# DaLi-Jack/G4Splat

Hardware: AMD Instinct MI355X
Metric: rasterized Gaussians/s fwd+bwd @1600x1200 (higher is better)
Workload: dtype f32

## Files before the change

g4splat_amd/csrc/api.hip:

```cpp
#include <stdarg.h>
#include <stdio.h>
#include <stdlib.h>
#include <string.h>

#include <atomic>
#include <mutex>
#include <vector>

#include "g4s_internal.h"

using namespace g4s;

namespace {
thread_local char t_err[512] = "";
}

namespace g4s {
void clear_error() { t_err[0] = 0; }
int fail(int code, const char* fmt, ...) {
    va_list ap;
    va_start(ap, fmt);
    vsnprintf(t_err, sizeof(t_err), fmt, ap);
    va_end(ap);
    return code;
// ... 267 lines not shown
        geom = align_ptr(geom);
        float* rec = (float*)(geom + GL.rec);
        uint32_t* tiles_touched = (uint32_t*)(geom + GL.tiles_touched);
        uint32_t* keys_a = (uint32_t*)(geom + GL.keys_a);
        uint32_t* keys_b = (uint32_t*)(geom + GL.keys_b);
        uint32_t* vals_a = (uint32_t*)(geom + GL.vals_a);
        uint32_t* vals_b = (uint32_t*)(geom + GL.vals_b);
        uint32_t* block_sums = (uint32_t*)(geom + GL.block_sums);
        uint32_t* block_offs = (uint32_t*)(geom + GL.block_offs);
        uint32_t* d_total = (uint32_t*)(geom + GL.total);
        int* const radii = c.radii ? c.radii : (int*)(geom + GL.internal_radii);

        PreprocessArgs pa{};
        pa.P = P; pa.D = c.D; pa.M = c.M; pa.W = c.width; pa.H = c.height; pa.tiles_x = tiles_x; pa.tiles_y = tiles_y;
        pa.means3D = c.means3D; pa.scales = c.scales; pa.rotations = c.rotations; pa.opacities = c.opacities; pa.shs = c.shs;
        pa.transMat_precomp = c.transMat_precomp; pa.colors_precomp = c.colors_precomp;
        pa.viewmatrix = c.viewmatrix; pa.projmatrix = c.projmatrix; pa.cam_pos = c.cam_pos;
        pa.scale_modifier = c.scale_modifier;
        pa.shs_rest = c.shs_rest;
        pa.sh_vec16 = (c.shs != nullptr && c.shs_rest == nullptr && c.M == 16 && !misaligned(c.shs, 16));
        pa.no_fastpath = opt(OPT_NO_FASTPATH) != 0;
        pa.rec = rec; pa.clamped = (uint8_t*)(geom + GL.clamped); pa.tiles_touched = tiles_touched; pa.radii = radii;
        pa.tight_rect = (uint2*)(geom + GL.tight_rect);
        uint32_t* const k_first = presized ? keys_b : keys_a;
        uint32_t* const k_other = presized ? keys_a : keys_b;
        uint32_t* const v_first = presized ? vals_b : vals_a;
        uint32_t* const v_other = presized ? vals_a : vals_b;
        pa.depth_keys = k_other;
        pa.ref_block_sums = (uint32_t*)(geom + GL.ref_block_sums);
        pa.idx_block_sums = (uint32_t*)(geom + GL.idx_block_sums);
        pa.vis_block_sums = (uint32_t*)(geom + GL.vis_block_sums);
        pa.key_min_blocks = (uint32_t*)(geom + GL.key_min_blocks);
        pa.key_max_blocks = (uint32_t*)(geom + GL.key_max_blocks);
        { ProfScope ps(PF_PREPROCESS_FWD, stream); launch_preprocess_fwd(pa, stream); }
        CHECK_LAUNCH("preprocess_fwd");

        uint32_t* idx_block_offs = (uint32_t*)(geom + GL.idx_block_offs);
        uint32_t* vis_block_offs = (uint32_t*)(geom + GL.vis_block_offs);
        uint32_t* h_total = nullptr;
        uint32_t* h_total_dev = nullptr;
        hipEvent_t totals_ready = nullptr;
        if (!presized) {
            h_total = pinned_word();
            h_total_dev = h_total ? pinned_word_device(h_total) : nullptr;
            if (!h_total || !h_total_dev) return fail(G4S_ERR_HIP, "hipHostMalloc / hipHostGetDevicePointer failed");
            totals_ready = readback_event();
            if (!totals_ready) return fail(G4S_ERR_HIP, "hipEventCreate failed");
        }
        { ProfScope ps(PF_COUNT_SCAN, stream);
          launch_scan_totals(pa.idx_block_sums, idx_block_offs, pa.ref_block_sums, pa.vis_block_sums, vis_block_offs,
                             d_total, GL.nblocks, ranges, tiles * 2, stream, presized ? (uint32_t)c.capacity : 0xFFFFFFFFu,
                             h_total_dev, presized ? c.status_dev : nullptr, pa.key_min_blocks, pa.key_max_blocks); }
        CHECK_LAUNCH("scan totals");
        if (!presized) {
            HIP_TRY(hipEventRecord(totals_ready, stream));
        }

        const uint32_t* d_V = d_total + 2;
        const uint32_t* d_key_min = d_total + 5;
        uint32_t* sort_hist = (uint32_t*)(geom + GL.hist);
        uint32_t* sort_bins = (uint32_t*)(geom + GL.bin_total);
        int cur;
        {
            ProfScope ps(PF_DEPTH_SORT, stream);
            launch_slots_and_compact(P, tiles_touched, idx_block_offs, rec, k_other, vis_block_offs, k_first, v_first,
                                     GL.nblocks, stream);
            cur = presized ? radix_sort_u32_pairs(k_first, k_other, v_first, v_other, P, sort_hist, sort_bins, stream, d_V)
                           : radix_sort_depth_low(k_first, k_other, v_first, v_other, P, sort_hist, sort_bins, stream, d_V,
                                                  d_key_min);
        }
        CHECK_LAUNCH("depth sort");

        int R_binned, V_emit, nblocks_v;
        const uint32_t* d_counts = nullptr;
        const uint32_t* d_nbinned = nullptr;
        if (!presized) {
            HIP_TRY(hipEventSynchronize(totals_ready));
            if (h_total[1] > 0x7FFFFFFFu) return fail(G4S_ERR_INVALID_ARGUMENT, "num_rendered overflows int");
            R = (int)h_total[1];
            R_binned = (int)h_total[0];
            V_emit = (int)h_total[2];
            nblocks_v = (V_emit + 255) / 256;
            if (V_emit > 0 && ((uint64_t)h_total[4] - h_total[3]) >> DEPTH_SORT_LOW_BITS) {
                ProfScope ps(PF_DEPTH_SORT, stream);
// ... 294 lines not shown
```

g4splat_amd/csrc/binning.hip:

```cpp
#include "g4s_internal.h"
#include "g4s_device.h"

namespace g4s {


template <typename K>
__device__ __forceinline__ uint32_t radix_digit(K key, uint32_t base, int shift, uint32_t mask) {
    return (uint32_t)((K)(key - (K)base) >> shift) & mask;
}

template <typename K, int ITEMS, int BITS>
__global__ void __launch_bounds__(256) radix_hist_kernel(const K* __restrict__ keys, int n, int shift, uint32_t mask,
                                                         uint32_t* __restrict__ hist, int nblocks,
                                                         const uint32_t* __restrict__ d_n,
                                                         const uint32_t* __restrict__ key_base) {
    constexpr int BINS = 1 << BITS;
    __shared__ uint32_t h[BINS];
    constexpr int TK = 256 * ITEMS;
    const int block = (int)blockIdx.x;
    if (d_n != nullptr) {
        n = (int)*d_n;
        nblocks = (n + TK - 1) / TK;
        if (block >= nblocks) return;
    }
// ... 202 lines not shown
    return cur ^ 1;
}

int radix_sort_u64_keys(uint64_t* a, uint64_t* b, int n, int begin_bit, int end_bit, uint32_t* hist,
                        uint32_t* bin_total, hipStream_t s, const uint32_t* d_n) {
    if (n <= 0 || end_bit <= begin_bit) return 0;
    const int bits = end_bit - begin_bit, passes = (bits + 7) / 8, per = (bits + passes - 1) / passes;
    int cur = 0;
    for (int shift = begin_bit; shift < end_bit; shift += per) {
        const int nb = per < end_bit - shift ? per : end_bit - shift;
        if (cur == 0)
            radix_pass<uint64_t, false, SORT_ITEMS_U64>(a, b, nullptr, nullptr, n, shift, nb, hist, bin_total, s, d_n);
        else
            radix_pass<uint64_t, false, SORT_ITEMS_U64>(b, a, nullptr, nullptr, n, shift, nb, hist, bin_total, s, d_n);
        cur ^= 1;
    }
    return cur;
}


__global__ void __launch_bounds__(256) count_block_sums_kernel(int P, const uint32_t* __restrict__ gidx,
                                                               const uint32_t* __restrict__ tiles_touched,
                                                               uint32_t* __restrict__ block_sums,
                                                               uint32_t* __restrict__ rank_local,
                                                               const uint32_t* __restrict__ d_n) {
    __shared__ uint32_t sm4[4];
    if (d_n != nullptr) {
        P = (int)*d_n;
        if ((int)(blockIdx.x * 256) >= P) return;
    }
    const int r = (int)(blockIdx.x * 256 + threadIdx.x);
    uint32_t c = 0;
    if (r < P) c = tiles_touched[gidx[r]];
    uint32_t total;
    const uint32_t local = block256_excl_scan_u32(c, sm4, &total);
    if (r < P) rank_local[r] = local;
    if (threadIdx.x == 0) block_sums[blockIdx.x] = total;
}

__global__ void __launch_bounds__(1024) scan_block_sums_kernel(int nblocks, const uint32_t* __restrict__ a_sums,
                                                               uint32_t* __restrict__ a_offs,
                                                               const uint32_t* __restrict__ b_sums,
                                                               uint32_t* __restrict__ b_offs,
                                                               const uint32_t* __restrict__ ref_sums,
                                                               uint32_t* __restrict__ total_a, uint32_t* __restrict__ total_b,
                                                               uint32_t* __restrict__ zero_ptr, int zero_words,
                                                               const uint32_t* __restrict__ d_n, uint32_t capacity,
                                                               uint32_t* __restrict__ host_out,
                                                               uint32_t* __restrict__ status_out,
                                                               const uint32_t* __restrict__ kmin_blocks,
                                                               const uint32_t* __restrict__ kmax_blocks) {
    __shared__ uint32_t wa[16], wb[16], wr[16], wlo[16], whi[16];
    const int t = (int)threadIdx.x;
    for (int i = t; i < zero_words; i += 1024) zero_ptr[i] = 0u;
    if (d_n != nullptr) nblocks = (int)((*d_n + 255u) / 256u);
    const int seg = (nblocks + 1023) / 1024;
    const int b = imin_(nblocks, t * seg), e = imin_(nblocks, b + seg);
    uint32_t sa = 0, sb = 0, sr = 0, klo = 0xFFFFFFFFu, khi = 0u;
    for (int i = b; i < e; i++) {
        sa += a_sums[i];
        if (b_sums) sb += b_sums[i];
        if (ref_sums) sr += ref_sums[i];
        if (kmin_blocks) {
            klo = min(klo, kmin_blocks[i]);
            khi = max(khi, kmax_blocks[i]);
        }
    }
    if (kmin_blocks) {
        klo = ~wave_max_u32_full_wave(~klo);
        khi = wave_max_u32_full_wave(khi);
    }
    const uint32_t ia = wave_incl_scan_u32(sa), ib = wave_incl_scan_u32(sb), ir = wave_incl_scan_u32(sr);
    if ((t & 63) == 63) {
        wa[t >> 6] = ia;
        wb[t >> 6] = ib;
        wr[t >> 6] = ir;
        wlo[t >> 6] = klo;
        whi[t >> 6] = khi;
    }
    __syncthreads();
    uint32_t base_a = 0, base_b = 0, all_a = 0, all_b = 0, all_r = 0;
    for (int w = 0; w < 16; w++) {
        if (w < (t >> 6)) { base_a += wa[w]; base_b += wb[w]; }
        all_a += wa[w];
        all_b += wb[w];
        all_r += wr[w];
    }
    uint32_t run_a = base_a + ia - sa, run_b = base_b + ib - sb;
    for (int i = b; i < e; i++) {
        a_offs[i] = run_a;
        run_a += a_sums[i];
        if (b_sums) { b_offs[i] = run_b; run_b += b_sums[i]; }
    }
    if (t == 0) {
        total_a[0] = all_a;
        total_a[1] = all_r;
        if (kmin_blocks) {
            uint32_t lo = 0xFFFFFFFFu, hi = 0u;
            for (int w = 0; w < 16; w++) { lo = min(lo, wlo[w]); hi = max(hi, whi[w]); }
            if (lo > hi) lo = hi = 0u;
            total_a[5] = lo;
            total_a[6] = hi;
            if (host_out != nullptr) { host_out[3] = lo; host_out[4] = hi; }
        }
        if (b_sums) {
            total_b[0] = all_b;
            total_b[1] = all_a < capacity ? all_a : capacity;
            total_b[2] = all_a > capacity ? 1u : 0u;
        }
        if (status_out != nullptr) {
            status_out[0] = all_r;
            status_out[1] = all_a;
            status_out[2] = all_b;
            status_out[3] = all_a > capacity ? 1u : 0u;
        }
        if (host_out != nullptr) {
            host_out[0] = all_a;
            host_out[1] = all_r;
            host_out[2] = all_b;
        }
    }
}

void launch_count_scan(int P, const uint32_t* gidx_sorted, const uint32_t* tiles_touched, uint32_t* block_sums,
                       uint32_t* block_offs, uint32_t* rank_local, uint32_t* total, int nblocks, hipStream_t s,
                       const uint32_t* d_n) {
    hipLaunchKernelGGL(count_block_sums_kernel, dim3(nblocks), dim3(256), 0, s, P, gidx_sorted, tiles_touched,
                       block_sums, rank_local, d_n);
    hipLaunchKernelGGL(scan_block_sums_kernel, dim3(1), dim3(1024), 0, s, nblocks, block_sums, block_offs,
                       (const uint32_t*)nullptr, (uint32_t*)nullptr, (const uint32_t*)nullptr, total, (uint32_t*)nullptr,
                       (uint32_t*)nullptr, 0, d_n, 0xFFFFFFFFu, (uint32_t*)nullptr, (uint32_t*)nullptr,
                       (const uint32_t*)nullptr, (const uint32_t*)nullptr);
}

constexpr int EMIT_SLOTS = 1024;
__global__ void __launch_bounds__(256) emit_kernel(int V, uint32_t R_b, int tiles_x,
                                                   const uint32_t* __restrict__ gidx,
                                                   const uint32_t* __restrict__ block_offs, int nblocks_v,
                                                   const uint32_t* __restrict__ rank_local,
                                                   const uint2* __restrict__ tight_rect,
                                                   uint64_t* __restrict__ entries, uint8_t* __restrict__ qhit,
                                                   uint8_t* __restrict__ rec_flag,
                                                   const uint32_t* __restrict__ d_counts) {
    __shared__ uint32_t s_off[EMIT_SLOTS + 4];
    __shared__ uint32_t s_idx[EMIT_SLOTS + 4];
    __shared__ uint32_t s_rect[EMIT_SLOTS + 4];
    __shared__ uint32_t s_rect2[EMIT_SLOTS + 4];
    __shared__ uint32_t s_nr;
    const int t = (int)threadIdx.x;
    if (d_counts != nullptr) {
        V = (int)d_counts[0];
        R_b = d_counts[1];
        nblocks_v = (V + 255) / 256;
    }
    const uint32_t w0 = blockIdx.x * (uint32_t)EMIT_SLOTS;
    if (w0 >= R_b) return;
    const uint32_t w1 = min(w0 + (uint32_t)EMIT_SLOTS, R_b);
    {
        const uint32_t o = w0 + 4u * (uint32_t)t;
        if (o + 4u <= w1) {
            *reinterpret_cast<uint32_t*>(qhit + o) = 0u;
            *reinterpret_cast<uint32_t*>(rec_flag + o) = 0u;
        } else {
            for (uint32_t i = o; i < w1; i++) { qhit[i] = 0; rec_flag[i] = 0; }
        }
    }
    if (t == 0) s_nr = 0;
    int lo = 0, n = nblocks_v;
    while (n > 1) {
        const int S = (n + 255) / 256;
        const int j = lo + t * S;
        const int c = __syncthreads_count(t * S < n && block_offs[j] <= w0);
        lo += (c - 1) * S;
        n = imin_(S, n - (c - 1) * S);
    }
    const int g = lo;
    const uint32_t goff = block_offs[g];
    int r_first;
    {
        const int r = 256 * g + t;
        const int c = __syncthreads_count(r < V && goff + rank_local[r] <= w0);
        r_first = 256 * g + c - 1;
    }
    for (int i = t; i <= EMIT_SLOTS; i += 256) {
        const int r = r_first + i;
        if (r >= V) break;
        const uint32_t off = block_offs[r >> 8] + rank_local[r];
        if (off >= w1) break;
        const uint32_t idx = gidx[r];
        const uint2 tr = tight_rect[idx];
        s_off[i] = off;
        s_idx[i] = idx;
        s_rect[i] = tr.x;
        s_rect2[i] = tr.y;
        atomicMax(&s_nr, (uint32_t)i + 1u);
    }
    __syncthreads();
    const int nr = (int)s_nr;
    const int steps = 32 - __builtin_clz((uint32_t)nr | 1u);
    for (uint32_t o = w0 + (uint32_t)t; o < w1; o += 256) {
        int a = 0, b = nr - 1;
        for (int it = 0; it < steps; it++) {
            const int mid = (a + b + 1) >> 1;
            if (s_off[mid] <= o) a = mid; else b = mid - 1;
        }
        const uint32_t k = o - s_off[a];
        const uint32_t w = s_rect2[a];
        const uint32_t rx0 = s_rect[a] & 0xFFFFu, ry0 = s_rect[a] >> 16;
        const uint32_t ty = k / w, tx = k - ty * w;
        const uint64_t tile = (uint64_t)((ry0 + ty) * (uint32_t)tiles_x + rx0 + tx);
        entries[o] = (tile << ENTRY_TILE_SHIFT) | (uint64_t)s_idx[a];
    }
}

__global__ void __launch_bounds__(256) slots_and_compact_kernel(int P, const uint32_t* __restrict__ tiles_touched,
                                                                const uint32_t* __restrict__ idx_block_offs,
                                                                float* __restrict__ rec,
                                                                const uint32_t* __restrict__ depth_keys,
                                                                const uint32_t* __restrict__ vis_block_offs,
                                                                uint32_t* __restrict__ keys_out,
                                                                uint32_t* __restrict__ idx_out) {
    __shared__ uint32_t sm4[4], sm4b[4];
    const int idx = (int)(blockIdx.x * 256 + threadIdx.x);
    const uint32_t c = idx < P ? tiles_touched[idx] : 0u;
    uint32_t total;
    const uint32_t slot = block256_excl_scan_u32(c, sm4, &total);
    const uint32_t local = block256_excl_scan_u32(c > 0 ? 1u : 0u, sm4b, &total);
    if (c > 0) {
        rec[(size_t)idx * REC_FLOATS + 2] = __uint_as_float(idx_block_offs[blockIdx.x] + slot);
        const uint32_t dst = vis_block_offs[blockIdx.x] + local;
        keys_out[dst] = depth_keys[idx];
        idx_out[dst] = (uint32_t)idx;
    }
}
void launch_slots_and_compact(int P, const uint32_t* tiles_touched, const uint32_t* idx_block_offs, float* rec,
                              const uint32_t* depth_keys, const uint32_t* vis_block_offs, uint32_t* keys_out,
                              uint32_t* idx_out, int nblocks, hipStream_t s) {
    hipLaunchKernelGGL(slots_and_compact_kernel, dim3(nblocks), dim3(256), 0, s, P, tiles_touched, idx_block_offs, rec,
                       depth_keys, vis_block_offs, keys_out, idx_out);
}

void launch_scan_totals(const uint32_t* idx_block_sums, uint32_t* idx_block_offs, const uint32_t* ref_block_sums,
                        const uint32_t* vis_block_sums, uint32_t* vis_block_offs, uint32_t* total, int nblocks,
                        uint32_t* zero_ptr, int zero_words, hipStream_t s, uint32_t capacity, uint32_t* host_out,
                        uint32_t* status_out, const uint32_t* key_min_blocks, const uint32_t* key_max_blocks) {
    hipLaunchKernelGGL(scan_block_sums_kernel, dim3(1), dim3(1024), 0, s, nblocks, idx_block_sums, idx_block_offs,
                       vis_block_sums, vis_block_offs, ref_block_sums, total, total + 2, zero_ptr, zero_words,
                       (const uint32_t*)nullptr, capacity, host_out, status_out, key_min_blocks, key_max_blocks);
}

void launch_emit(int V, uint32_t R_b, int tiles_x, const uint32_t* gidx_sorted, const uint32_t* block_offs,
                 int nblocks_v, const uint32_t* rank_local, const uint2* tight_rect, uint64_t* entries,
                 uint8_t* qhit, uint8_t* rec_flag, hipStream_t s, const uint32_t* d_counts) {
    if (R_b == 0) return;
    hipLaunchKernelGGL(emit_kernel, dim3((R_b + EMIT_SLOTS - 1) / EMIT_SLOTS), dim3(256), 0, s, V, R_b, tiles_x,
                       gidx_sorted, block_offs, nblocks_v, rank_local, tight_rect, entries, qhit, rec_flag, d_counts);
}

__global__ void __launch_bounds__(256) tile_ranges_kernel(int R, const uint64_t* __restrict__ entries,
                                                          uint32_t* __restrict__ ranges, const uint32_t* __restrict__ d_n) {
    if (d_n != nullptr) R = (int)*d_n;
    const int i0 = (int)(blockIdx.x * 256 + threadIdx.x) * 4;
    if (i0 >= R) return;
    uint64_t e[4];
    if (i0 + 4 <= R) {
        const ulonglong2 a = *reinterpret_cast<const ulonglong2*>(entries + i0);
        const ulonglong2 b = *reinterpret_cast<const ulonglong2*>(entries + i0 + 2);
        e[0] = a.x; e[1] = a.y; e[2] = b.x; e[3] = b.y;
    } else {
#pragma unroll
        for (int k = 0; k < 4; k++) e[k] = entries[i0 + k < R ? i0 + k : R - 1];
    }
    uint32_t prev = i0 > 0 ? entry_tile(entries[i0 - 1]) : 0xFFFFFFFFu;
#pragma unroll
    for (int k = 0; k < 4; k++) {
        const int i = i0 + k;
        if (i >= R) break;
        const uint32_t cur = entry_tile(e[k]);
        if (i == 0) {
            ranges[2 * cur] = 0;
        } else if (cur != prev) {
            ranges[2 * prev + 1] = (uint32_t)i;
            ranges[2 * cur] = (uint32_t)i;
        }
        if (i == R - 1) ranges[2 * cur + 1] = (uint32_t)R;
        prev = cur;
    }
}

constexpr int ORDER_BUCKETS = 2048;
__global__ void __launch_bounds__(1024) tile_order_kernel(int tiles, const uint32_t* __restrict__ ranges,
                                                          uint32_t* __restrict__ order, uint32_t* __restrict__ zero_word) {
    __shared__ uint32_t hist[ORDER_BUCKETS];
    __shared__ uint32_t wsum[16];
    const int t = (int)threadIdx.x;
    if (t == 0 && zero_word != nullptr) *zero_word = 0u;
    for (int i = t; i < ORDER_BUCKETS; i += 1024) hist[i] = 0;
    __syncthreads();
    auto bucket = [](uint32_t n) {
        const uint32_t b = n >> 2;
        return (uint32_t)(ORDER_BUCKETS - 1) - (b < (uint32_t)(ORDER_BUCKETS - 1) ? b : (uint32_t)(ORDER_BUCKETS - 1));
    };
    for (int i = t; i < tiles; i += 1024) atomicAdd(&hist[bucket(ranges[2 * i + 1] - ranges[2 * i])], 1u);
    __syncthreads();
    const uint32_t h0 = hist[2 * t], h1 = hist[2 * t + 1];
    const uint32_t inc = wave_incl_scan_u32(h0 + h1);
    if ((t & 63) == 63) wsum[t >> 6] = inc;
    __syncthreads();
    uint32_t base = 0;
    for (int w = 0; w < (t >> 6); w++) base += wsum[w];
    const uint32_t ex = base + inc - (h0 + h1);
    __syncthreads();
    hist[2 * t] = ex;
    hist[2 * t + 1] = ex + h0;
    __syncthreads();
    for (int i = t; i < tiles; i += 1024) order[atomicAdd(&hist[bucket(ranges[2 * i + 1] - ranges[2 * i])], 1u)] = (uint32_t)i;
}
void launch_tile_order(int tiles, const uint32_t* ranges, uint32_t* tile_order, hipStream_t s, uint32_t* zero_word) {
    hipLaunchKernelGGL(tile_order_kernel, dim3(1), dim3(1024), 0, s, tiles, ranges, tile_order, zero_word);
}

void launch_tile_ranges(int R, const uint64_t* entries, uint32_t* ranges, hipStream_t s, const uint32_t* d_n) {
    if (R <= 0) return;
    hipLaunchKernelGGL(tile_ranges_kernel, dim3((R + 1023) / 1024), dim3(256), 0, s, R, entries, ranges, d_n);
}

}
```

g4splat_amd/csrc/g4s_device.h:

```cpp
#pragma once
#include <hip/hip_runtime.h>
#include <stdint.h>

#include "g4s_internal.h"

namespace g4s {

constexpr int WAVE = 64;

__device__ __forceinline__ int lane_id() { return (int)(threadIdx.x & 63); }

template <int CTRL, int ROW_MASK = 0xF, int BANK_MASK = 0xF>
__device__ __forceinline__ float dpp_f32(float v) {
    return __builtin_bit_cast(
        float, __builtin_amdgcn_update_dpp(0, __builtin_bit_cast(int, v), CTRL, ROW_MASK, BANK_MASK, false));
}
template <int CTRL, int ROW_MASK = 0xF, int BANK_MASK = 0xF>
__device__ __forceinline__ uint32_t dpp_u32(uint32_t v) {
    return (uint32_t)__builtin_amdgcn_update_dpp(0, (int)v, CTRL, ROW_MASK, BANK_MASK, false);
}

__device__ __forceinline__ void acc_fma(float& acc, float a, float b) { asm volatile("v_fmac_f32 %0, %1, %2" : "+v"(acc) : "v"(a), "v"(b)); }
__device__ __forceinline__ void acc_add(float& acc, float a) { asm volatile("v_add_f32 %0, %0, %1" : "+v"(acc) : "v"(a)); }
__device__ __forceinline__ void acc_sub(float& acc, float a) { asm volatile("v_sub_f32 %0, %0, %1" : "+v"(acc) : "v"(a)); }
// ... 92 lines not shown
        "v_permlane16_swap_b32 %3, %7"
        : "+v"(s0), "+v"(s1), "+v"(s2), "+v"(s3), "+v"(s4), "+v"(s5), "+v"(s6), "+v"(s7));
    const float r0 = s0 + s4, r1 = s1 + s5, r2 = s2 + s6, r3 = s3 + s7;
    const float k01 = b3 ? r1 : r0, g01 = b3 ? r0 : r1;
    const float k23 = b3 ? r3 : r2, g23 = b3 ? r2 : r3;
    const float x01 = k01 + dpp_f32<0x128>(g01);
    const float x23 = k23 + dpp_f32<0x128>(g23);
    const float k = b2 ? x23 : x01, g = b2 ? x01 : x23;
    float y = k + dpp_f32<0x141>(g);
    y += dpp_f32<0xB1>(y);
    y += dpp_f32<0x4E>(y);
    asm volatile("" : "+v"(y));
    return y;
}

__device__ __forceinline__ uint32_t wave_sum_u32(uint32_t v) {
    return (uint32_t)__builtin_amdgcn_readlane((int)wave_sum_to_lane63(v), 63);
}
__device__ __forceinline__ uint32_t wave_max_u32(uint32_t v) {
    for (int off = 32; off >= 1; off >>= 1) {
        uint32_t o = (uint32_t)__shfl_xor((int)v, off, 64);
        v = v > o ? v : o;
    }
    return v;
}
__device__ __forceinline__ uint32_t wave_max_u32_full_wave(uint32_t v) {
    v = max(v, dpp_u32<0xB1>(v));
    v = max(v, dpp_u32<0x4E>(v));
    v = max(v, dpp_u32<0x124>(v));
    v = max(v, dpp_u32<0x128>(v));
    v = max(v, dpp_u32<0x142, 0xA>(v));
    v = max(v, dpp_u32<0x143, 0xC>(v));
    return (uint32_t)__builtin_amdgcn_readlane((int)v, 63);
}

__device__ __forceinline__ uint32_t wave_incl_scan_u32(uint32_t v) {
    const int l = lane_id();
    for (int off = 1; off < 64; off <<= 1) {
        uint32_t o = (uint32_t)__shfl_up((int)v, off, 64);
        if (l >= off) v += o;
    }
    return v;
}

__device__ __forceinline__ uint64_t lanes_below_mask() {
    return (1ull << lane_id()) - 1ull;
}

__device__ __forceinline__ uint32_t block256_excl_scan_u32(uint32_t v, uint32_t* smem4, uint32_t* block_total) {
    const int w = (int)(threadIdx.x >> 6);
    uint32_t inc = wave_incl_scan_u32(v);
    __syncthreads();
    if (lane_id() == 63) smem4[w] = inc;
    __syncthreads();
    uint32_t s0 = smem4[0], s1 = smem4[1], s2 = smem4[2], s3 = smem4[3];
    uint32_t base = (w > 0 ? s0 : 0) + (w > 1 ? s1 : 0) + (w > 2 ? s2 : 0);
    *block_total = s0 + s1 + s2 + s3;
    return base + inc - v;
}

__device__ __forceinline__ int sat_int(float v) { return (int)v; }

struct F3 {
    float x, y, z;
};
__device__ __forceinline__ F3 mk3(float x, float y, float z) { return F3{x, y, z}; }
// ... 171 lines not shown
```

g4splat_amd/csrc/g4s_internal.h:

```cpp
#pragma once
#include <hip/hip_runtime.h>
#include <stddef.h>
#include <stdint.h>

#include "../../include/g4s_rasterizer.h"

namespace g4s {

constexpr int TILE = 16;
constexpr int REC_FLOATS = 32;
constexpr int REC_QUADS = REC_FLOATS / 4;
constexpr int BLEND_QUADS = 5;
constexpr int GRAD_FLOATS = 18;
constexpr int GRAD_STRIDE = 20;
__host__ __device__ inline void box_quadrants(float lo, float hi, int extent, uint32_t& q0, uint32_t& q1) {
    const float l = ceilf(lo), h = floorf(hi);
    const float top = (float)(extent - 1);
    q0 = 1u;
    q1 = 0u;
    if (!(l <= h) || !(h >= 0.0f) || !(l <= top)) return;
    q0 = (l > 0.0f ? (uint32_t)l : 0u) >> 3;
    q1 = (h < top ? (uint32_t)h : (uint32_t)(extent - 1)) >> 3;
}
constexpr uint32_t CULLED_KEY = 0xFFFFFFFFu;
// ... 96 lines not shown
int fail(int code, const char* fmt, ...);
int finish(hipError_t e, const char* what);
int stage_done(const char* what, hipStream_t s, bool debug = false);
inline bool misaligned(const void* p, size_t a) { return p != nullptr && ((size_t)p % a) != 0; }

enum ProfId { PF_PREPROCESS_FWD, PF_DEPTH_SORT, PF_COUNT_SCAN, PF_EMIT, PF_TILE_SORT, PF_TILE_RANGES, PF_BLEND_FWD,
              PF_BLEND_BWD, PF_PREPROCESS_BWD, PF_MAPS_FWD, PF_MAPS_BWD, PF_PHOTO_LOSS, PF_ADAM, PF_GEO_REG, PF_COUNT };
struct ProfScope {
    int id; hipStream_t s; hipEvent_t a = nullptr, b = nullptr; bool on = false;
    ProfScope(int id_, hipStream_t s_);
    ~ProfScope();
};


struct PreprocessArgs {
    int P, D, M, W, H, tiles_x, tiles_y;
    uint32_t* ref_block_sums;
    uint32_t* idx_block_sums;
    uint32_t* vis_block_sums;
    uint32_t* key_min_blocks;
    uint32_t* key_max_blocks;
    const float *means3D, *scales, *rotations, *opacities, *shs, *transMat_precomp, *colors_precomp;
    const float *viewmatrix, *projmatrix, *cam_pos;
    float scale_modifier;
    bool sh_vec16;
    bool no_fastpath;
    const float* shs_rest;
    float* rec;
    uint8_t* clamped;
    uint32_t* tiles_touched;
    uint2* tight_rect;
    int* radii;
    uint32_t* depth_keys;
};
void launch_preprocess_fwd(const PreprocessArgs& a, hipStream_t s);

int radix_sort_u32_pairs(uint32_t* keys_a, uint32_t* keys_b, uint32_t* vals_a, uint32_t* vals_b, int n,
                         uint32_t* hist, uint32_t* bin_total, hipStream_t s, const uint32_t* d_n = nullptr);
int radix_sort_depth_low(uint32_t* keys_a, uint32_t* keys_b, uint32_t* vals_a, uint32_t* vals_b, int n, uint32_t* hist,
                         uint32_t* bin_total, hipStream_t s, const uint32_t* d_n, const uint32_t* key_min);
int radix_sort_depth_top(uint32_t* keys_a, uint32_t* keys_b, uint32_t* vals_a, uint32_t* vals_b, int n, int cur,
                         uint32_t* hist, uint32_t* bin_total, hipStream_t s, const uint32_t* d_n, const uint32_t* key_min);
int radix_sort_u64_keys(uint64_t* a, uint64_t* b, int n, int begin_bit, int end_bit, uint32_t* hist,
                        uint32_t* bin_total, hipStream_t s, const uint32_t* d_n = nullptr);

void launch_count_scan(int P, const uint32_t* gidx_sorted, const uint32_t* tiles_touched, uint32_t* block_sums,
                       uint32_t* block_offs, uint32_t* rank_local, uint32_t* total, int nblocks, hipStream_t s,
                       const uint32_t* d_n = nullptr);
void launch_scan_totals(const uint32_t* idx_block_sums, uint32_t* idx_block_offs, const uint32_t* ref_block_sums,
                        const uint32_t* vis_block_sums, uint32_t* vis_block_offs, uint32_t* total, int nblocks,
                        uint32_t* zero_ptr, int zero_words, hipStream_t s, uint32_t capacity = 0xFFFFFFFFu,
                        uint32_t* host_out = nullptr, uint32_t* status_out = nullptr,
                        const uint32_t* key_min_blocks = nullptr, const uint32_t* key_max_blocks = nullptr);
void launch_slots_and_compact(int P, const uint32_t* tiles_touched, const uint32_t* idx_block_offs, float* rec,
                              const uint32_t* depth_keys, const uint32_t* vis_block_offs, uint32_t* keys_out,
                              uint32_t* idx_out, int nblocks, hipStream_t s);
void launch_emit(int V, uint32_t R_b, int tiles_x, const uint32_t* gidx_sorted, const uint32_t* block_offs,
                 int nblocks_v, const uint32_t* rank_local, const uint2* tight_rect, uint64_t* entries,
                 uint8_t* qhit, uint8_t* rec_flag, hipStream_t s, const uint32_t* d_counts);
void launch_tile_ranges(int R, const uint64_t* entries, uint32_t* ranges, hipStream_t s, const uint32_t* d_n = nullptr);
void launch_tile_order(int tiles, const uint32_t* ranges, uint32_t* tile_order, hipStream_t s, uint32_t* zero_word = nullptr);

struct BlendFwdArgs {
    int W, H, tiles_x, tiles_y;
    const uint32_t* ranges;
    const uint32_t* tile_order;
// ... 67 lines not shown
```

g4splat_amd/csrc/preprocess.hip:

```cpp
#include "g4s_internal.h"
#include "g4s_device.h"

namespace g4s {

__constant__ float c_SH_C2[5] = {1.0925484305920792f, -1.0925484305920792f, 0.31539156525252005f,
                                 -1.0925484305920792f, 0.5462742152960396f};
__constant__ float c_SH_C3[7] = {-0.5900435899266435f, 2.890611442640554f, -0.4570457994644658f,
                                 0.3731763325901154f,  -0.4570457994644658f, 1.445305721320277f,
                                 -0.5900435899266435f};
#define SH_C0 0.28209479177387814f
#define SH_C1 0.4886025119029199f

__device__ __forceinline__ void compute_transmat(F3 p, float sx, float sy, float mod, const float* R,
                                                 const float* proj, int W, int H, float* T) {
    const float s0 = mod * sx, s1 = mod * sy;
    const float Mrow[3][4] = {{R[0] * s0, R[1] * s0, R[2] * s0, 0.0f},
                              {R[3] * s1, R[4] * s1, R[5] * s1, 0.0f},
                              {p.x, p.y, p.z, 1.0f}};
    const float hw = (float)((float)W / 2.0), cw = (float)((float)(W - 1) / 2.0);
    const float hh = (float)((float)H / 2.0), ch = (float)((float)(H - 1) / 2.0);
#pragma unroll
    for (int r = 0; r < 3; r++) {
        float c[4];
#pragma unroll
// ... 255 lines not shown
            r[c] = r[c] - SH_C1 * y * sh[3 + c] + SH_C1 * z * sh[6 + c] - SH_C1 * x * sh[9 + c];
        if (deg > 1) {
            const float xx = x * x, yy = y * y, zz = z * z, xy = x * y, yz = y * z, xz = x * z;
#pragma unroll
            for (int c = 0; c < 3; c++)
                r[c] = r[c] + c_SH_C2[0] * xy * sh[12 + c] + c_SH_C2[1] * yz * sh[15 + c] +
                       c_SH_C2[2] * (2.0f * zz - xx - yy) * sh[18 + c] + c_SH_C2[3] * xz * sh[21 + c] +
                       c_SH_C2[4] * (xx - yy) * sh[24 + c];
            if (deg > 2) {
#pragma unroll
                for (int c = 0; c < 3; c++)
                    r[c] = r[c] + c_SH_C3[0] * y * (3.0f * xx - yy) * sh[27 + c] + c_SH_C3[1] * xy * z * sh[30 + c] +
                           c_SH_C3[2] * y * (4.0f * zz - xx - yy) * sh[33 + c] +
                           c_SH_C3[3] * z * (2.0f * zz - 3.0f * xx - 3.0f * yy) * sh[36 + c] +
                           c_SH_C3[4] * x * (4.0f * zz - xx - yy) * sh[39 + c] +
                           c_SH_C3[5] * z * (xx - yy) * sh[42 + c] + c_SH_C3[6] * x * (xx - 3.0f * yy) * sh[45 + c];
            }
        }
    }
    clamp_bits = 0;
#pragma unroll
    for (int c = 0; c < 3; c++) {
        r[c] += 0.5f;
        if (r[c] < 0) clamp_bits |= (1u << c);
        rgb[c] = fmaxf(r[c], 0.0f);
    }
}

template <int SH_MODE>
__global__ void __launch_bounds__(256) __attribute__((amdgpu_waves_per_eu(5, 5))) preprocess_fwd_kernel(PreprocessArgs a) {
    __shared__ __attribute__((aligned(16))) float s_cert[4][64 * CERT_SLOT_WORDS];
    __shared__ uint32_t s_cert_fail[4][64];
    const int idx = (int)(blockIdx.x * 256 + threadIdx.x);
    const bool in_range = idx < a.P;
    int radius_out = 0;
    uint32_t touched_ref = 0, touched = 0, key = CULLED_KEY, clamp_bits = 0;
    float T[9], cx, cy, opa, rgb[3];
    F3 normal;
    float4 box;
    int tx0, ty0, tx1, ty1;
    SplatAffine af;
    bool want = false;

    if (in_range) {
        const F3 p = mk3(a.means3D[3 * idx], a.means3D[3 * idx + 1], a.means3D[3 * idx + 2]);
        const F3 p_view = xform_point_4x3(p, a.viewmatrix);
        if (p_view.z > 0.2f) {
            if (a.transMat_precomp == nullptr) {
                float R[9];
                const float4 q = reinterpret_cast<const float4*>(a.rotations)[idx];
                const float2 sc = reinterpret_cast<const float2*>(a.scales)[idx];
                quat_to_rotmat(q, R);
                compute_transmat(p, sc.x, sc.y, a.scale_modifier, R, a.projmatrix, a.W, a.H, T);
                normal = xform_vec_4x3(mk3(R[6], R[7], R[8]), a.viewmatrix);
            } else {
#pragma unroll
                for (int i = 0; i < 9; i++) T[i] = a.transMat_precomp[9 * (size_t)idx + i];
                normal = mk3(0.0f, 0.0f, 1.0f);
            }
            const float cosv = -((p_view.x * normal.x + p_view.y * normal.y) + p_view.z * normal.z);
            if (cosv != 0) {
                const float mult = cosv > 0 ? 1.0f : -1.0f;
                normal = mk3(mult * normal.x, mult * normal.y, mult * normal.z);
                float ex, ey;
                if (compute_aabb(T, 3.0f, cx, cy, ex, ey)) {
                    const float radius = ceilf(fmaxf(ex, ey));
// ... 754 lines not shown
```

Baseline: 268.6 million.

## Rework binning scans, emit lookup, tile order, and move range zeroing into preprocess

Zeroing of the tile ranges buffer moves out of the single-block scan_totals kernel and into the grid-wide preprocess kernel. The block-sum scan is now chunked and wave-parallel with DPP scans instead of serial per-thread segments. The emit kernel replaces its per-output binary search with an owner map built in shared memory plus a running max, and writes entries as vectorized stores. Count-scan and tile-order kernels use full-wave DPP scans and keep loaded values in registers. Together these aim to cut serial work and latency in the small binning kernels, at the cost of more shared memory and register use and a more complex emit index computation.

```diff
diff --git a/g4splat_amd/csrc/api.hip b/g4splat_amd/csrc/api.hip
--- a/g4splat_amd/csrc/api.hip
+++ b/g4splat_amd/csrc/api.hip
@@ -323,6 +323,7 @@
         pa.vis_block_sums = (uint32_t*)(geom + GL.vis_block_sums);
         pa.key_min_blocks = (uint32_t*)(geom + GL.key_min_blocks);
         pa.key_max_blocks = (uint32_t*)(geom + GL.key_max_blocks);
+        pa.zero_ptr = ranges; pa.zero_words = (uint32_t)tiles * 2u;
         { ProfScope ps(PF_PREPROCESS_FWD, stream); launch_preprocess_fwd(pa, stream); }
         CHECK_LAUNCH("preprocess_fwd");
 
@@ -340,7 +341,7 @@
         }
         { ProfScope ps(PF_COUNT_SCAN, stream);
           launch_scan_totals(pa.idx_block_sums, idx_block_offs, pa.ref_block_sums, pa.vis_block_sums, vis_block_offs,
-                             d_total, GL.nblocks, ranges, tiles * 2, stream, presized ? (uint32_t)c.capacity : 0xFFFFFFFFu,
+                             d_total, GL.nblocks, nullptr, 0, stream, presized ? (uint32_t)c.capacity : 0xFFFFFFFFu,
                              h_total_dev, presized ? c.status_dev : nullptr, pa.key_min_blocks, pa.key_max_blocks); }
         CHECK_LAUNCH("scan totals");
         if (!presized) {
diff --git a/g4splat_amd/csrc/binning.hip b/g4splat_amd/csrc/binning.hip
--- a/g4splat_amd/csrc/binning.hip
+++ b/g4splat_amd/csrc/binning.hip
@@ -258,12 +258,16 @@
     const int r = (int)(blockIdx.x * 256 + threadIdx.x);
     uint32_t c = 0;
     if (r < P) c = tiles_touched[gidx[r]];
-    uint32_t total;
-    const uint32_t local = block256_excl_scan_u32(c, sm4, &total);
-    if (r < P) rank_local[r] = local;
-    if (threadIdx.x == 0) block_sums[blockIdx.x] = total;
-}
-
+    const int w = (int)(threadIdx.x >> 6);
+    const uint32_t inc = wave_incl_scan_u32_full_wave(c);
+    if (lane_id() == 63) sm4[w] = inc;
+    __syncthreads();
+    const uint32_t s0 = sm4[0], s1 = sm4[1], s2 = sm4[2], s3 = sm4[3];
+    if (r < P) rank_local[r] = (w > 0 ? s0 : 0u) + (w > 1 ? s1 : 0u) + (w > 2 ? s2 : 0u) + inc - c;
+    if (threadIdx.x == 0) block_sums[blockIdx.x] = (s0 + s1) + (s2 + s3);
+}
+
+constexpr int SCAN_CHUNKS = 8;
 __global__ void __launch_bounds__(1024) scan_block_sums_kernel(int nblocks, const uint32_t* __restrict__ a_sums,
                                                                uint32_t* __restrict__ a_offs,
                                                                const uint32_t* __restrict__ b_sums,
@@ -276,54 +280,97 @@
                                                                uint32_t* __restrict__ status_out,
                                                                const uint32_t* __restrict__ kmin_blocks,
                                                                const uint32_t* __restrict__ kmax_blocks) {
-    __shared__ uint32_t wa[16], wb[16], wr[16], wlo[16], whi[16];
-    const int t = (int)threadIdx.x;
+    __shared__ uint32_t s_wa[16 * SCAN_CHUNKS], s_wb[16 * SCAN_CHUNKS];
+    __shared__ uint32_t wr[16], wlo[16], whi[16];
+    const int t = (int)threadIdx.x, lane = t & 63, w = __builtin_amdgcn_readfirstlane(t >> 6);
     for (int i = t; i < zero_words; i += 1024) zero_ptr[i] = 0u;
     if (d_n != nullptr) nblocks = (int)((*d_n + 255u) / 256u);
-    const int seg = (nblocks + 1023) / 1024;
-    const int b = imin_(nblocks, t * seg), e = imin_(nblocks, b + seg);
-    uint32_t sa = 0, sb = 0, sr = 0, klo = 0xFFFFFFFFu, khi = 0u;
-    for (int i = b; i < e; i++) {
-        sa += a_sums[i];
-        if (b_sums) sb += b_sums[i];
-        if (ref_sums) sr += ref_sums[i];
-        if (kmin_blocks) {
-            klo = min(klo, kmin_blocks[i]);
-            khi = max(khi, kmax_blocks[i]);
-        }
-    }
-    if (kmin_blocks) {
-        klo = ~wave_max_u32_full_wave(~klo);
-        khi = wave_max_u32_full_wave(khi);
-    }
-    const uint32_t ia = wave_incl_scan_u32(sa), ib = wave_incl_scan_u32(sb), ir = wave_incl_scan_u32(sr);
-    if ((t & 63) == 63) {
-        wa[t >> 6] = ia;
-        wb[t >> 6] = ib;
-        wr[t >> 6] = ir;
-        wlo[t >> 6] = klo;
-        whi[t >> 6] = khi;
-    }
-    __syncthreads();
-    uint32_t base_a = 0, base_b = 0, all_a = 0, all_b = 0, all_r = 0;
-    for (int w = 0; w < 16; w++) {
-        if (w < (t >> 6)) { base_a += wa[w]; base_b += wb[w]; }
-        all_a += wa[w];
-        all_b += wb[w];
-        all_r += wr[w];
-    }
-    uint32_t run_a = base_a + ia - sa, run_b = base_b + ib - sb;
-    for (int i = b; i < e; i++) {
-        a_offs[i] = run_a;
-        run_a += a_sums[i];
-        if (b_sums) { b_offs[i] = run_b; run_b += b_sums[i]; }
-    }
+    uint32_t all_a = 0, all_b = 0, sr = 0, klo = 0xFFFFFFFFu, khi = 0u;
+    const uint32_t* pb = b_sums != nullptr ? b_sums : a_sums;
+    const uint32_t* pr = ref_sums != nullptr ? ref_sums : a_sums;
+    const uint32_t* plo = kmin_blocks != nullptr ? kmin_blocks : a_sums;
+    const uint32_t* phi = kmin_blocks != nullptr ? kmax_blocks : a_sums;
+    int first = 0;
+    do {
+        const bool last = first + 1024 * SCAN_CHUNKS >= nblocks;
+        uint32_t va[SCAN_CHUNKS], vb[SCAN_CHUNKS], vr[SCAN_CHUNKS], vlo[SCAN_CHUNKS], vhi[SCAN_CHUNKS];
+#pragma unroll
+        for (int c = 0; c < SCAN_CHUNKS; c++) {
+            const int i = first + 1024 * c + t;
+            const int ic = i < nblocks ? i : 0;
+            va[c] = a_sums[ic];
+            vb[c] = pb[ic];
+            vr[c] = pr[ic];
+            vlo[c] = plo[ic];
+            vhi[c] = phi[ic];
+        }
+#pragma unroll
+        for (int c = 0; c < SCAN_CHUNKS; c++) {
+            const bool in = first + 1024 * c + t < nblocks;
+            va[c] = in ? va[c] : 0u;
+            vb[c] = in && b_sums != nullptr ? vb[c] : 0u;
+            vr[c] = in && ref_sums != nullptr ? vr[c] : 0u;
+            vlo[c] = in && kmin_blocks != nullptr ? vlo[c] : 0xFFFFFFFFu;
+            vhi[c] = in && kmin_blocks != nullptr ? vhi[c] : 0u;
+        }
+        uint32_t ia[SCAN_CHUNKS], ib[SCAN_CHUNKS];
+#pragma unroll
+        for (int c = 0; c < SCAN_CHUNKS; c++) {
+            ia[c] = ib[c] = 0u;
+            if (first + 1024 * c < nblocks) {
+                ia[c] = wave_incl_scan_u32_full_wave(va[c]);
+                if (b_sums != nullptr) ib[c] = wave_incl_scan_u32_full_wave(vb[c]);
+                sr += vr[c];
+                klo = min(klo, vlo[c]);
+                khi = max(khi, vhi[c]);
+            }
+            if (lane == 63) {
+                s_wa[16 * c + w] = ia[c];
+                s_wb[16 * c + w] = ib[c];
+            }
+        }
+        if (last) {
+            const uint32_t ir = wave_sum_to_lane63(sr);
+            if (kmin_blocks) {
+                klo = ~wave_max_u32_full_wave(~klo);
+                khi = wave_max_u32_full_wave(khi);
+            }
+            if (lane == 63) {
+                wr[w] = ir;
+                wlo[w] = klo;
+                whi[w] = khi;
+            }
+        }
+        __syncthreads();
+        const uint32_t a0 = s_wa[2 * lane], a1 = s_wa[2 * lane + 1], b0 = s_wb[2 * lane], b1 = s_wb[2 * lane + 1];
+        const uint32_t inc_a = wave_incl_scan_u32_full_wave(a0 + a1), inc_b = wave_incl_scan_u32_full_wave(b0 + b1);
+        const uint32_t ex_a = inc_a - (a0 + a1), ex_b = inc_b - (b0 + b1);
+#pragma unroll
+        for (int c = 0; c < SCAN_CHUNKS; c++) {
+            const int i = first + 1024 * c + t;
+            if (first + 1024 * c >= nblocks) break;
+            const int src = (16 * c + w) >> 1;
+            const uint32_t pa = (uint32_t)__builtin_amdgcn_readlane((int)(w & 1 ? ex_a + a0 : ex_a), src);
+            const uint32_t pb = (uint32_t)__builtin_amdgcn_readlane((int)(w & 1 ? ex_b + b0 : ex_b), src);
+            if (i < nblocks) {
+                a_offs[i] = all_a + pa + (ia[c] - va[c]);
+                if (b_sums != nullptr) b_offs[i] = all_b + pb + (ib[c] - vb[c]);
+            }
+        }
+        all_a += (uint32_t)__builtin_amdgcn_readlane((int)inc_a, 63);
+        all_b += (uint32_t)__builtin_amdgcn_readlane((int)inc_b, 63);
+        first += 1024 * SCAN_CHUNKS;
+        if (last) break;
+        __syncthreads();
+    } while (true);
     if (t == 0) {
+        uint32_t all_r = 0;
+        for (int k = 0; k < 16; k++) all_r += wr[k];
         total_a[0] = all_a;
         total_a[1] = all_r;
         if (kmin_blocks) {
             uint32_t lo = 0xFFFFFFFFu, hi = 0u;
-            for (int w = 0; w < 16; w++) { lo = min(lo, wlo[w]); hi = max(hi, whi[w]); }
+            for (int k = 0; k < 16; k++) { lo = min(lo, wlo[k]); hi = max(hi, whi[k]); }
             if (lo > hi) lo = hi = 0u;
             total_a[5] = lo;
             total_a[6] = hi;
@@ -360,6 +407,8 @@
 }
 
 constexpr int EMIT_SLOTS = 1024;
+constexpr int EMIT_PROBES = 8;
+constexpr int EMIT_GROUPS = 5;
 __global__ void __launch_bounds__(256) emit_kernel(int V, uint32_t R_b, int tiles_x,
                                                    const uint32_t* __restrict__ gidx,
                                                    const uint32_t* __restrict__ block_offs, int nblocks_v,
@@ -368,12 +417,10 @@
                                                    uint64_t* __restrict__ entries, uint8_t* __restrict__ qhit,
                                                    uint8_t* __restrict__ rec_flag,
                                                    const uint32_t* __restrict__ d_counts) {
-    __shared__ uint32_t s_off[EMIT_SLOTS + 4];
-    __shared__ uint32_t s_idx[EMIT_SLOTS + 4];
-    __shared__ uint32_t s_rect[EMIT_SLOTS + 4];
-    __shared__ uint32_t s_rect2[EMIT_SLOTS + 4];
-    __shared__ uint32_t s_nr;
-    const int t = (int)threadIdx.x;
+    __shared__ __attribute__((aligned(16))) uint4 s_rank[EMIT_SLOTS];
+    __shared__ __attribute__((aligned(8))) uint16_t s_owner[EMIT_SLOTS];
+    __shared__ uint32_t s_cnt[4], s_wmax[4];
+    const int t = (int)threadIdx.x, lane = t & 63, wv = t >> 6;
     if (d_counts != nullptr) {
         V = (int)d_counts[0];
         R_b = d_counts[1];
@@ -391,51 +438,85 @@
             for (uint32_t i = o; i < w1; i++) { qhit[i] = 0; rec_flag[i] = 0; }
         }
     }
-    if (t == 0) s_nr = 0;
+    *reinterpret_cast<uint2*>(&s_owner[4 * t]) = make_uint2(0u, 0u);
     int lo = 0, n = nblocks_v;
-    while (n > 1) {
+    while (n > 256 * EMIT_PROBES - (EMIT_GROUPS - 1)) {
         const int S = (n + 255) / 256;
         const int j = lo + t * S;
         const int c = __syncthreads_count(t * S < n && block_offs[j] <= w0);
         lo += (c - 1) * S;
         n = imin_(S, n - (c - 1) * S);
     }
-    const int g = lo;
-    const uint32_t goff = block_offs[g];
-    int r_first;
+    n = imin_(n + (EMIT_GROUPS - 1), nblocks_v - lo);
+    uint32_t c_le = 0, c_lt = 0;
     {
-        const int r = 256 * g + t;
-        const int c = __syncthreads_count(r < V && goff + rank_local[r] <= w0);
-        r_first = 256 * g + c - 1;
-    }
-    for (int i = t; i <= EMIT_SLOTS; i += 256) {
-        const int r = r_first + i;
-        if (r >= V) break;
-        const uint32_t off = block_offs[r >> 8] + rank_local[r];
-        if (off >= w1) break;
-        const uint32_t idx = gidx[r];
-        const uint2 tr = tight_rect[idx];
-        s_off[i] = off;
-        s_idx[i] = idx;
-        s_rect[i] = tr.x;
-        s_rect2[i] = tr.y;
-        atomicMax(&s_nr, (uint32_t)i + 1u);
-    }
-    __syncthreads();
-    const int nr = (int)s_nr;
-    const int steps = 32 - __builtin_clz((uint32_t)nr | 1u);
-    for (uint32_t o = w0 + (uint32_t)t; o < w1; o += 256) {
-        int a = 0, b = nr - 1;
-        for (int it = 0; it < steps; it++) {
-            const int mid = (a + b + 1) >> 1;
-            if (s_off[mid] <= o) a = mid; else b = mid - 1;
-        }
-        const uint32_t k = o - s_off[a];
-        const uint32_t w = s_rect2[a];
-        const uint32_t rx0 = s_rect[a] & 0xFFFFu, ry0 = s_rect[a] >> 16;
-        const uint32_t ty = k / w, tx = k - ty * w;
+        uint32_t v[EMIT_PROBES];
+#pragma unroll
+        for (int k = 0; k < EMIT_PROBES; k++) v[k] = t + 256 * k < n ? block_offs[lo + t + 256 * k] : 0xFFFFFFFFu;
+#pragma unroll
+        for (int k = 0; k < EMIT_PROBES; k++) {
+            const bool in = t + 256 * k < n;
+            c_le += (uint32_t)__popcll(__ballot(in && v[k] <= w0));
+            c_lt += (uint32_t)__popcll(__ballot(in && v[k] < w1));
+        }
+    }
+    if (lane == 0) s_cnt[wv] = c_le | (c_lt << 16);
+    __syncthreads();
+    const uint32_t cnt = (s_cnt[0] + s_cnt[1]) + (s_cnt[2] + s_cnt[3]);
+    const int g = lo + (int)(cnt & 0xFFFFu) - 1;
+    const int ngroups = imin_((int)(cnt >> 16) - (int)(cnt & 0xFFFFu) + 1, EMIT_GROUPS);
+    uint32_t off[EMIT_GROUPS], idx[EMIT_GROUPS];
+#pragma unroll
+    for (int m = 0; m < EMIT_GROUPS; m++) {
+        const int r = 256 * (g + m) + t;
+        const bool in = m < ngroups && r < V;
+        const uint32_t goff = in ? block_offs[g + m] : 0u;
+        off[m] = in ? goff + rank_local[r] : 0xFFFFFFFFu;
+        idx[m] = in ? gidx[r] : 0u;
+    }
+    const int c0 = __syncthreads_count(off[0] <= w0);
+#pragma unroll
+    for (int m = 0; m < EMIT_GROUPS; m++) {
+        const int i = 256 * m + t - (c0 - 1);
+        if (off[m] < w1 && i >= 0 && i < EMIT_SLOTS) {
+            const uint2 tr = tight_rect[idx[m]];
+            s_rank[i] = make_uint4(off[m], idx[m], tr.x, tr.y);
+            s_owner[max(off[m], w0) - w0] = (uint16_t)i;
+        }
+    }
+    __syncthreads();
+    const uint2 mk = *reinterpret_cast<const uint2*>(&s_owner[4 * t]);
+    uint32_t own[4] = {mk.x & 0xFFFFu, mk.x >> 16, mk.y & 0xFFFFu, mk.y >> 16};
+    own[1] = max(own[1], own[0]);
+    own[2] = max(own[2], own[1]);
+    own[3] = max(own[3], own[2]);
+    const uint32_t run = wave_incl_max_u32_full_wave(own[3]);
+    if (lane == 63) s_wmax[wv] = run;
+    uint32_t before = (uint32_t)__shfl_up((int)run, 1, 64);
+    if (lane == 0) before = 0u;
+    __syncthreads();
+#pragma unroll
+    for (int k = 0; k < 3; k++)
+        if (k < wv) before = max(before, s_wmax[k]);
+    const uint32_t o0 = w0 + 4u * (uint32_t)t;
+    uint64_t e[4];
+#pragma unroll
+    for (int k = 0; k < 4; k++) {
+        const uint4 rk = s_rank[max(own[k], before)];
+        const uint32_t inst = o0 + (uint32_t)k - rk.x;
+        const uint32_t w = rk.w;
+        const uint32_t rx0 = rk.z & 0xFFFFu, ry0 = rk.z >> 16;
+        const uint32_t ty = inst / w, tx = inst - ty * w;
         const uint64_t tile = (uint64_t)((ry0 + ty) * (uint32_t)tiles_x + rx0 + tx);
-        entries[o] = (tile << ENTRY_TILE_SHIFT) | (uint64_t)s_idx[a];
+        e[k] = (tile << ENTRY_TILE_SHIFT) | (uint64_t)rk.y;
+    }
+    if (o0 + 4u <= w1) {
+        *reinterpret_cast<ulonglong2*>(entries + o0) = make_ulonglong2(e[0], e[1]);
+        *reinterpret_cast<ulonglong2*>(entries + o0 + 2) = make_ulonglong2(e[2], e[3]);
+    } else {
+#pragma unroll
+        for (int k = 0; k < 4; k++)
+            if (o0 + (uint32_t)k < w1) entries[o0 + k] = e[k];
     }
 }
 
@@ -449,9 +530,20 @@
     __shared__ uint32_t sm4[4], sm4b[4];
     const int idx = (int)(blockIdx.x * 256 + threadIdx.x);
     const uint32_t c = idx < P ? tiles_touched[idx] : 0u;
-    uint32_t total;
-    const uint32_t slot = block256_excl_scan_u32(c, sm4, &total);
-    const uint32_t local = block256_excl_scan_u32(c > 0 ? 1u : 0u, sm4b, &total);
+    const int w = (int)(threadIdx.x >> 6);
+    const uint32_t inc_c = wave_incl_scan_u32_full_wave(c), inc_v = wave_incl_scan_u32_full_wave(c > 0 ? 1u : 0u);
+    if (lane_id() == 63) {
+        sm4[w] = inc_c;
+        sm4b[w] = inc_v;
+    }
+    __syncthreads();
+    uint32_t slot = inc_c - c, local = inc_v - (c > 0 ? 1u : 0u);
+#pragma unroll
+    for (int k = 0; k < 3; k++)
+        if (k < w) {
+            slot += sm4[k];
+            local += sm4b[k];
+        }
     if (c > 0) {
         rec[(size_t)idx * REC_FLOATS + 2] = __uint_as_float(idx_block_offs[blockIdx.x] + slot);
         const uint32_t dst = vis_block_offs[blockIdx.x] + local;
@@ -515,32 +607,54 @@
 }
 
 constexpr int ORDER_BUCKETS = 2048;
+constexpr int ORDER_HELD = 8;
 __global__ void __launch_bounds__(1024) tile_order_kernel(int tiles, const uint32_t* __restrict__ ranges,
                                                           uint32_t* __restrict__ order, uint32_t* __restrict__ zero_word) {
     __shared__ uint32_t hist[ORDER_BUCKETS];
     __shared__ uint32_t wsum[16];
     const int t = (int)threadIdx.x;
     if (t == 0 && zero_word != nullptr) *zero_word = 0u;
-    for (int i = t; i < ORDER_BUCKETS; i += 1024) hist[i] = 0;
-    __syncthreads();
     auto bucket = [](uint32_t n) {
         const uint32_t b = n >> 2;
         return (uint32_t)(ORDER_BUCKETS - 1) - (b < (uint32_t)(ORDER_BUCKETS - 1) ? b : (uint32_t)(ORDER_BUCKETS - 1));
     };
-    for (int i = t; i < tiles; i += 1024) atomicAdd(&hist[bucket(ranges[2 * i + 1] - ranges[2 * i])], 1u);
+    const uint2* pairs = reinterpret_cast<const uint2*>(ranges);
+    uint2 held[ORDER_HELD];
+#pragma unroll
+    for (int k = 0; k < ORDER_HELD; k++) {
+        const int i = t + 1024 * k;
+        held[k] = i < tiles ? pairs[i] : make_uint2(0u, 0u);
+    }
+    for (int i = t; i < ORDER_BUCKETS; i += 1024) hist[i] = 0;
+    __syncthreads();
+    uint32_t bk[ORDER_HELD];
+#pragma unroll
+    for (int k = 0; k < ORDER_HELD; k++) {
+        bk[k] = bucket(held[k].y - held[k].x);
+        if (t + 1024 * k < tiles) atomicAdd(&hist[bk[k]], 1u);
+    }
+    for (int i = t + 1024 * ORDER_HELD; i < tiles; i += 1024) {
+        const uint2 r = pairs[i];
+        atomicAdd(&hist[bucket(r.y - r.x)], 1u);
+    }
     __syncthreads();
     const uint32_t h0 = hist[2 * t], h1 = hist[2 * t + 1];
-    const uint32_t inc = wave_incl_scan_u32(h0 + h1);
+    const uint32_t inc = wave_incl_scan_u32_full_wave(h0 + h1);
     if ((t & 63) == 63) wsum[t >> 6] = inc;
     __syncthreads();
     uint32_t base = 0;
     for (int w = 0; w < (t >> 6); w++) base += wsum[w];
     const uint32_t ex = base + inc - (h0 + h1);
-    __syncthreads();
     hist[2 * t] = ex;
     hist[2 * t + 1] = ex + h0;
     __syncthreads();
-    for (int i = t; i < tiles; i += 1024) order[atomicAdd(&hist[bucket(ranges[2 * i + 1] - ranges[2 * i])], 1u)] = (uint32_t)i;
+#pragma unroll
+    for (int k = 0; k < ORDER_HELD; k++)
+        if (t + 1024 * k < tiles) order[atomicAdd(&hist[bk[k]], 1u)] = (uint32_t)(t + 1024 * k);
+    for (int i = t + 1024 * ORDER_HELD; i < tiles; i += 1024) {
+        const uint2 r = pairs[i];
+        order[atomicAdd(&hist[bucket(r.y - r.x)], 1u)] = (uint32_t)i;
+    }
 }
 void launch_tile_order(int tiles, const uint32_t* ranges, uint32_t* tile_order, hipStream_t s, uint32_t* zero_word) {
     hipLaunchKernelGGL(tile_order_kernel, dim3(1), dim3(1024), 0, s, tiles, ranges, tile_order, zero_word);
diff --git a/g4splat_amd/csrc/g4s_device.h b/g4splat_amd/csrc/g4s_device.h
--- a/g4splat_amd/csrc/g4s_device.h
+++ b/g4splat_amd/csrc/g4s_device.h
@@ -148,6 +148,25 @@
     v = max(v, dpp_u32<0x142, 0xA>(v));
     v = max(v, dpp_u32<0x143, 0xC>(v));
     return (uint32_t)__builtin_amdgcn_readlane((int)v, 63);
+}
+
+__device__ __forceinline__ uint32_t wave_incl_scan_u32_full_wave(uint32_t v) {
+    v += dpp_u32<0x111>(v);
+    v += dpp_u32<0x112>(v);
+    v += dpp_u32<0x114>(v);
+    v += dpp_u32<0x118>(v);
+    v += dpp_u32<0x142, 0xA>(v);
+    v += dpp_u32<0x143, 0xC>(v);
+    return v;
+}
+__device__ __forceinline__ uint32_t wave_incl_max_u32_full_wave(uint32_t v) {
+    v = max(v, dpp_u32<0x111>(v));
+    v = max(v, dpp_u32<0x112>(v));
+    v = max(v, dpp_u32<0x114>(v));
+    v = max(v, dpp_u32<0x118>(v));
+    v = max(v, dpp_u32<0x142, 0xA>(v));
+    v = max(v, dpp_u32<0x143, 0xC>(v));
+    return v;
 }
 
 __device__ __forceinline__ uint32_t wave_incl_scan_u32(uint32_t v) {
diff --git a/g4splat_amd/csrc/g4s_internal.h b/g4splat_amd/csrc/g4s_internal.h
--- a/g4splat_amd/csrc/g4s_internal.h
+++ b/g4splat_amd/csrc/g4s_internal.h
@@ -152,6 +152,8 @@
     uint2* tight_rect;
     int* radii;
     uint32_t* depth_keys;
+    uint32_t* zero_ptr;
+    uint32_t zero_words;
 };
 void launch_preprocess_fwd(const PreprocessArgs& a, hipStream_t s);
 
diff --git a/g4splat_amd/csrc/preprocess.hip b/g4splat_amd/csrc/preprocess.hip
--- a/g4splat_amd/csrc/preprocess.hip
+++ b/g4splat_amd/csrc/preprocess.hip
@@ -311,6 +311,7 @@
     __shared__ __attribute__((aligned(16))) float s_cert[4][64 * CERT_SLOT_WORDS];
     __shared__ uint32_t s_cert_fail[4][64];
     const int idx = (int)(blockIdx.x * 256 + threadIdx.x);
+    for (uint32_t i = (uint32_t)idx; i < a.zero_words; i += gridDim.x * 256u) a.zero_ptr[i] = 0u;
     const bool in_range = idx < a.P;
     int radius_out = 0;
     uint32_t touched_ref = 0, touched = 0, key = CULLED_KEY, clamp_bits = 0;
```

New measurement: 272.2 million, median of 6. 1.01x the previous value.
